# RobinWitch/SynTalker

Measured on AMD Instinct MI355X. Metric: denoising-steps/sec (128-frame clips), higher is better.
Workload: dtype bf16

## Files before the change

### include/syn_hip.h

```cpp
#ifndef SYN_HIP_H
#define SYN_HIP_H

#include <stddef.h>
#include <stdint.h>

#ifdef __cplusplus
extern "C" {
#endif

#define SYN_ABI_VERSION 9
#define SYN_D        512
#define SYN_T        32
#define SYN_C        1536
#define SYN_FF       1024
#define SYN_HEADS    4
#define SYN_LAYERS   8

int         syn_version(void);
const char* syn_last_error(void);

typedef struct syn_layer {
    const float* ln1_g;  const float* ln1_b;
    const void*  w_qkv;
    const void*  w_proj; const float* b_proj;
// ... 495 lines not shown
int syn_vq_train_wgrad(const void* dy_bf16, int32_t ldy, const void* x_bf16, int32_t ldx, float* dw, float* db, int32_t clips, int32_t t_in,
                       int32_t t_out, int32_t cout, int32_t cin, int32_t taps, int32_t stride, int32_t dil, int32_t pad, int32_t up, int32_t relu_in,
                       void* stream);
int syn_vq_train_codebook_prep(const float* codebook, float* codebook_t, float* code_sq, void* stream);
int syn_vq_train_tile(const float* x, int32_t rows, const float* noise, float* codebook, float* code_sum, float* code_count, void* stream);
int syn_vq_train_quantize(const float* x_in, const float* codebook, const float* codebook_t, const float* code_sq, const float* gumbel, float temperature,
                          float* x_out, float* q_acc, void* q_bf16, float* resid_sum, int32_t* idx, float* sqerr, int32_t layer, int32_t first, int32_t rows,
                          void* stream);
int syn_vq_train_codebook_update(const float* x_in, const int32_t* idx, int32_t layer, int32_t rows, const float* noise, float mu, float one_minus_mu,
                                 float* codebook, float* code_sum, float* code_count, float* batch_count, void* stream);
int32_t syn_vq_train_loss_parts(int64_t rows, int32_t dim_padded);
int syn_vq_train_loss(const float* rec, const float* gt, int64_t rows, int32_t dim, int32_t dim_padded, int32_t kind, void* d_rec_bf16, float* parts,
                      void* stream);
int syn_vq_train_scalars(const float* parts, int32_t n_parts, int64_t count, const float* sqerr, int32_t groups, const float* batch_count, int32_t n_active,
                         int32_t rows, float commit_weight, float* out4, void* stream);

int syn_linear(const void* x_bf16, const void* w_packed, const float* bias, int32_t m_rows, int32_t n, int32_t k, float* y,
               void* stream);
int syn_linear_and_pack(const void* x_bf16, const void* w_packed, const float* bias, int32_t m_rows, int32_t n, int32_t k, float* y,
                        void* xt_packed, void* stream);
int syn_linear_pair(const void* x1_bf16, const void* w1_packed, int32_t m1, int32_t n1, int32_t k1, float* y1,
                    const void* x2_bf16, const void* w2_packed, int32_t m2, int32_t n2, int32_t k2, float* y2,
                    const float* bias_parts, int32_t part_rows, int32_t part_n, float* bias_grad, void* stream);
int syn_linear_res(const void* x_bf16, const void* w_packed, const float* bias, const float* residual, const float* row_scale,
                   int32_t rows_per_scale, int32_t m_rows, int32_t n, int32_t k, float* y, void* xt_packed, void* stream);
int syn_linear_gelu(const void* x_bf16, const void* w_packed, const float* bias, int32_t m_rows, int32_t n, int32_t k, float* y, void* y_gelu_bf16,
                    void* xt_packed, void* stream);

int syn_test_gemm(const void* x_bf16, const void* w_packed, const float* bias, int32_t m_rows, int32_t n, int32_t k,
                  int32_t m_tile, float* y, void* stream);
int syn_test_handoff(uint32_t* sync_320_zeroed, uint32_t* buf_8x4096, const float* stream, int64_t stream_n, uint32_t* stale_9_zeroed,
                     int32_t words, int32_t rounds, int32_t mode, void* stream_h);
int syn_test_mfma_rate(int32_t iters, float* out, int64_t* flops, void* stream);
int syn_test_attention(const void* q, const void* k, const void* vt, int32_t n_seq, void* o, void* stream);

void syn_debug_timing(long long* attn_buf, long long* mlp_buf);
void syn_debug_gemm_resident(int on);
void syn_debug_linear_tile(int rows);
void syn_debug_conv_terms(int mask);
void syn_debug_seq_skew(int units_of_64_cycles);
void syn_debug_seq_step(int step);

#ifdef __cplusplus
}
#endif
#endif
```

### syntalker_amd/csrc/syn_kernels.hip

```cpp
#include <hip/hip_runtime.h>
#include <stdint.h>
#include <stdio.h>
#include <stdlib.h>
#include <string.h>

#include "syn_hip.h"

typedef __attribute__((ext_vector_type(8))) __bf16 bf16x8;
typedef __attribute__((ext_vector_type(4))) __bf16 bf16x4;
typedef __attribute__((ext_vector_type(4))) float f32x4;

#define MFMA16(a, b, c) __builtin_amdgcn_mfma_f32_16x16x32_bf16((a), (b), (c), 0, 0, 0)

namespace {

constexpr int kThreads = 512;
constexpr int kKT = 64;
constexpr int kNT = 512;

enum Epi { EPI_PLAIN = 0, EPI_IN = 1, EPI_QKV = 2, EPI_RESID = 3, EPI_GELU = 4, EPI_OUT = 5 };

struct GArgs {
    const __bf16* X; long x_chunk_stride; int ldx; int x_rows;
    const uint4* W; int K; int M;
// ... 1798 lines not shown
        hipLaunchKernelGGL((k_gemm_pair<16, 2>), grid, dim3(kThreads), lds128, (hipStream_t)stream, p);
    } else if (g_gemm_resident == 1 && fits)
        hipLaunchKernelGGL((k_gemm_pair<16, 1>), grid, dim3(kThreads), (k1 > k2 ? k1 : k2) * 32, (hipStream_t)stream, p);
    else
        hipLaunchKernelGGL((k_gemm_pair<16, 0>), grid, dim3(kThreads), 2 * 32 * 128 + 1024, (hipStream_t)stream, p);
    return launched("k_gemm_pair launch");
}

void syn_debug_gemm_resident(int on) { g_gemm_resident = on; }
void syn_debug_linear_tile(int rows) { g_linear_mt = rows; }

int syn_test_handoff(uint32_t* sync_320_zeroed, uint32_t* buf_8x4096, const float* stream, int64_t stream_n, uint32_t* stale_9_zeroed,
                     int32_t words, int32_t rounds, int32_t mode, void* stream_h) {
    if (!sync_320_zeroed || !buf_8x4096 || !stale_9_zeroed || words <= 0 || words > 4096 || rounds <= 0 || mode < 0 || mode > 4)
        return fail_msg("syn_test_handoff: bad arguments");
    if (!latency_path_ok()) return fail_msg("syn_test_handoff: needs a 256-CU (8 XCD x 32) device");
    static OncePerDevice once;
    if (once.first()) { allow_lds(lat::k_handoff_stress, 96 * 1024); }
    lat::HArgs a;
    a.sync = sync_320_zeroed; a.buf = buf_8x4096; a.stream = stream; a.stream_n = stream_n; a.stale = stale_9_zeroed;
    a.words = words; a.rounds = rounds; a.mode = mode;
    hipLaunchKernelGGL(lat::k_handoff_stress, dim3(256), dim3(512), 96 * 1024, (hipStream_t)stream_h, a);
    return launched("k_handoff_stress launch");
}

int syn_test_mfma_rate(int32_t iters, float* out, int64_t* flops, void* stream) {
    if (iters <= 0 || !out) return fail_msg("syn_test_mfma_rate: bad arguments (out: 256 floats per CU)");
    static OncePerDevice once;
    if (once.first()) { allow_lds(seq::k_mfma_rate, seq::kLds); }
    const int cus = device_cus();
    hipLaunchKernelGGL(seq::k_mfma_rate, dim3(cus), dim3(seq::kThreads), seq::kLds, (hipStream_t)stream, out, iters);
    if (flops) *flops = (int64_t)cus * 4 * (int64_t)iters * 16 * 12 * (2LL * 32 * 32 * 16);
    return launched("k_mfma_rate launch");
}

int syn_test_attention(const void* q, const void* k, const void* vt, int32_t n_seq, void* o, void* stream) {
    if (!q || !k || !vt || !o || n_seq <= 0) return fail_msg("syn_test_attention: bad arguments");
    hipLaunchKernelGGL(k_attn, dim3(n_seq), dim3(256), 0, (hipStream_t)stream, (const __bf16*)q, (const __bf16*)k,
                       (const __bf16*)vt, (__bf16*)o, n_seq);
    return launched("k_attn launch");
}

int syn_rotary(const float* x, const float* cos_t, const float* sin_t, int32_t n_seq, int32_t inverse, float* y, void* stream) {
    if (!x || !cos_t || !sin_t || !y || n_seq <= 0) return fail_msg("syn_rotary: null pointer / empty batch");
    const long n_tok = (long)n_seq * SYN_T;
    hipLaunchKernelGGL(trn::k_rotary, dim3((unsigned)((n_tok * 64 + 255) / 256)), dim3(256), 0, (hipStream_t)stream, x, cos_t, sin_t, n_tok, inverse, y);
    return launched("k_rotary launch");
}

enum { ST_IN = 0, ST_QKV = 1, ST_ATTN = 2, ST_PROJ = 3, ST_FC1 = 4, ST_FC2 = 5, ST_COMBINE = 6, ST_OUT = 7, ST_N = 8 };

struct StageTimer {
    bool on = false;
    hipStream_t s = nullptr;
    hipEvent_t ev[64];
    int cls[64];
    int n = 0;
    void begin(hipStream_t st) { on = true; s = st; hipEventCreate(&ev[0]); hipEventRecord(ev[0], s); n = 1; }
    void mark(int c) {
        if (!on || n >= 64) return;
        hipEventCreate(&ev[n]); hipEventRecord(ev[n], s); cls[n] = c; ++n;
    }
};

static int g_seq_skew = -1, g_seq_dbg_step = 0;

// ... 245 lines not shown
```

### syntalker_amd/csrc/syn_seq.inc

```
namespace {
namespace seq {

typedef __attribute__((ext_vector_type(16))) float f32x16;
#define MFMA32(a, b, c) __builtin_amdgcn_mfma_f32_32x32x16_bf16((a), (b), (c), 0, 0, 0)

#ifndef SEQ_ABL
#define SEQ_ABL 0
#endif
#ifndef SEQ_ABL2
#define SEQ_ABL2 0
#endif
constexpr int kThreads = 256;
constexpr int kFragBytes = 1024;
#ifndef SEQ_CHUNK
#define SEQ_CHUNK 16
#endif
#ifndef SEQ_WIN
#define SEQ_WIN 4
#endif
#ifndef SEQ_SPREAD
#define SEQ_SPREAD 1
#endif
#ifndef SEQ_SCHED
#define SEQ_SCHED 0
#endif
constexpr int kChunkFrags = SEQ_CHUNK, kChunkBytes = kChunkFrags * kFragBytes;
constexpr int kPerWave = kChunkFrags / 4;
constexpr int kSlots = 80 / kChunkFrags, kLook = kSlots - 1;
constexpr int kRingBytes = kSlots * kChunkBytes;
constexpr int kBiasSet = 2048;
constexpr int kRingBase = 0;
constexpr int kBiasBase = kRingBytes;
constexpr int kSlabBase = kBiasBase + 2 * kBiasSet * 4;
constexpr int kSlabBytes = 4 * 4096;
constexpr int kLds = kSlabBase + 4 * kSlabBytes;
#if SEQ_CHUNK == 16
#define SEQ_WAIT_STEADY "s_waitcnt vmcnt(8)"
#define SEQ_WAIT_FIRST "s_waitcnt vmcnt(12)"
#else
#define SEQ_WAIT_STEADY "s_waitcnt vmcnt(14)"
#define SEQ_WAIT_FIRST "s_waitcnt vmcnt(16)"
#endif

struct QArgs {
    const char* tape; unsigned tape_chunks;
    const float* bias;
    const float* te; const float* rcos; const float* rsin;
    const float* cond; const int* t_model;
    const float* xt;
    const uint4* xb;
    const float* noise;
    const unsigned long long* rng; const float* coef; const int* t_coef;
    float* xn; uint4* xnb; float* x0;
    int R;
    int V;
    const float* cfg_w;
    int cfg_stride;
    int n_steps;
    int tm_stride, tc_stride;
    int wg0, n_wg;
    int dbg_step;
    unsigned skew;
    long long* dbg;
};

__device__ __forceinline__ void dma_frag(const char* src, unsigned lds_dst, unsigned lane16) {
    unsigned keep;
    asm volatile("s_mov_b32 %0, m0\n\t"
                 "s_mov_b32 m0, %2\n\t"
                 "s_nop 0\n\t"
                 "global_load_lds_dwordx4 %1, %3\n\t"
                 "s_mov_b32 m0, %0"
                 : "=&s"(keep) : "v"(lane16), "s"(lds_dst), "s"(src) : "memory");
}

template <int OFF>
__device__ __forceinline__ void dma_frag_at(const char* src, unsigned lds_dst, unsigned lane16) {
    asm volatile("s_mov_b32 m0, %1\n\t"
                 "s_nop 0\n\t"
                 "global_load_lds_dwordx4 %0, %2 offset:%c3"
                 :: "v"(lane16), "s"(lds_dst), "s"(src), "i"(OFF) : "memory");
}

#ifndef SEQ_DMA_POL
#define SEQ_DMA_POL 0
#endif
#if SEQ_DMA_POL == 1
#define SEQ_DMA_POLICY " nt"
#elif SEQ_DMA_POL == 2
#define SEQ_DMA_POLICY " sc1"
#elif SEQ_DMA_POL == 3
#define SEQ_DMA_POLICY " sc0"
#else
#define SEQ_DMA_POLICY ""
#endif
struct Ring {
    const char* tape;
    unsigned voff;
    unsigned dst;
    unsigned wq;
    unsigned voff0;
    unsigned lane16;
    unsigned cur, nxt;
    bf16x8 win[SEQ_WIN];
};
static_assert(SEQ_CHUNK == 16 && kPerWave == 4, "the pinned ring arithmetic below is written for 16-fragment chunks");

template <int OFF>
__device__ __forceinline__ void ring_dma(const Ring& r) {
    asm volatile("s_add_u32 m0, %1, %2\n\t"
                 "s_nop 0\n\t"
                 "global_load_lds_dwordx4 %0, %3 offset:%c4" SEQ_DMA_POLICY
                 :: "v"(r.voff), "s"(r.dst), "s"(r.wq), "s"(r.tape), "i"(OFF) : "memory", "scc");
}
__device__ __forceinline__ void ring_dma_i(const Ring& r, int i) {
    switch (i) {
        case 0: ring_dma<0>(r); break;
        case 1: ring_dma<1024>(r); break;
        case 2: ring_dma<2048>(r); break;
        default: ring_dma<3072>(r); break;
    }
}
__device__ __forceinline__ void ring_advance_dma(Ring& r) {
    const unsigned d = r.dst + kChunkBytes;
    r.dst = d == (unsigned)kRingBytes ? 0u : d;
    r.voff += kChunkBytes;
}
__device__ __forceinline__ void ring_next_base(Ring& r) {
    static_assert(kSlots == 5 && kRingBase == 0, "slot arithmetic");
    unsigned t = r.dst + 2 * kChunkBytes;
    t = t >= (unsigned)kRingBytes ? t - kRingBytes : t;
    r.nxt = r.lane16 + t;
}

__device__ __forceinline__ void bias_issue(const float* bias, const Ring& r, int set) {
    const char* src = reinterpret_cast<const char*>(bias + (size_t)set * kBiasSet) + r.wq / 2;
    const unsigned dst = kBiasBase + (set & 1) * (kBiasSet * 4) + r.wq / 2;
    dma_frag(src, dst, r.lane16);
    dma_frag(src + kFragBytes, dst + kFragBytes, r.lane16);
}

__device__ __forceinline__ void ring_boundary(Ring& r) {
    if (!(SEQ_ABL & 2)) {
        if (!(SEQ_ABL & 64)) asm volatile(SEQ_WAIT_STEADY ::: "memory");
        if (!(SEQ_ABL & 128)) __builtin_amdgcn_s_barrier();
    }
    r.cur = r.nxt;
}

__device__ __forceinline__ bf16x8 take(Ring& r, const char* lds, int& f) {
    if (f == 0) {
        const bf16x8 a = r.win[0];
        if (!(SEQ_ABL & 4)) r.win[0] = *reinterpret_cast<const bf16x8*>(lds + r.nxt + SEQ_WIN * kFragBytes);
        ring_boundary(r);
        __builtin_amdgcn_sched_barrier(0);
        f = 1;
        return a;
    }
    if (!(SEQ_ABL & 1) && (f & 3) == 2) ring_dma_i(r, f >> 2);
    if (f == 6) ring_next_base(r);
    if (f == 15) ring_advance_dma(r);
    const bf16x8 a = r.win[f & (SEQ_WIN - 1)];
    const int g = f + SEQ_WIN;
    if (!(SEQ_ABL & 4))
        r.win[f & (SEQ_WIN - 1)] = *reinterpret_cast<const bf16x8*>(lds + (g < kChunkFrags ? r.cur + g * kFragBytes : r.nxt + (g - kChunkFrags) * kFragBytes));
#if SEQ_SCHED == 0
    __builtin_amdgcn_sched_barrier(0);
#else
    __builtin_amdgcn_sched_group_barrier(0x100, 1, 0);
    __builtin_amdgcn_sched_group_barrier(0x008, 1, 0);
    __builtin_amdgcn_sched_group_barrier(0x002, SEQ_SCHED, 0);
#endif
    f = (f + 1) & (kChunkFrags - 1);
    return a;
}

__device__ __forceinline__ bf16x8 pack8(const f32x16& t, int c) {
    bf16x8 o;
#pragma unroll
    for (int e = 0; e < 8; ++e) o[e] = (__bf16)t[8 * c + e];
    return o;
}

__device__ __forceinline__ f32x16 zero16() {
    f32x16 z;
#pragma unroll
    for (int v = 0; v < 16; ++v) z[v] = 0.f;
// ... 22 lines not shown
    }
    return o;
}
__device__ __forceinline__ void slab_store(char* slab, int t, const f32x16& v) {
#pragma unroll
    for (int q = 0; q < 4; ++q)
        *reinterpret_cast<f32x4*>(slab + (t * 4 + q) * 1024) = f32x4{v[4 * q], v[4 * q + 1], v[4 * q + 2], v[4 * q + 3]};
}

__device__ __forceinline__ float xor32(float v) { return __shfl_xor(v, 32); }

__device__ __forceinline__ float gelu_fast(float x) {
    if (SEQ_ABL2 & 1) return x;
    const float x2 = fminf(x * x, 64.0f);
    float t = fmaf(1.0142633e-3f, x2, -1.0677573e-1f);
    t = fmaf(t, x2, -2.3011213f);
    const float e = __builtin_amdgcn_exp2f(x * t);
    return nopk(x * __builtin_amdgcn_rcpf(1.0f + e));
}

struct NoFill { __device__ __forceinline__ void operator()(int) const {} };

__device__ __forceinline__ void slab_load_half(const char* slab, int t, int half, f32x16& o) {
#pragma unroll
    for (int q = 2 * half; q < 2 * half + 2; ++q) {
        const f32x4 v = *reinterpret_cast<const f32x4*>(slab + (t * 4 + q) * 1024);
        o[4 * q] = v[0]; o[4 * q + 1] = v[1]; o[4 * q + 2] = v[2]; o[4 * q + 3] = v[3];
    }
}
__device__ __forceinline__ void slab_store_quad(char* slab, int t, int q, const f32x16& v) {
    *reinterpret_cast<f32x4*>(slab + (t * 4 + q) * 1024) = f32x4{v[4 * q], v[4 * q + 1], v[4 * q + 2], v[4 * q + 3]};
}

template <int KC, int SPLIT = 0, typename Opnd, typename Fill = NoFill>
__device__ __forceinline__ void wide_of(Ring& r, const char* lds, f32x16 (&h)[12], char* slab, Opnd opnd, Fill fill = Fill()) {
    static_assert(SPLIT >= 0 && SPLIT < KC && (SPLIT == 0 || 12 * SPLIT >= 20), "slab loads must fit in front of their first use");
    constexpr int kLoad0 = SPLIT ? 12 * SPLIT - 12 : 0;
    constexpr int kStore0 = KC > 1 ? 16 * (KC - 1) + 4 : 16 * KC;
    f32x16 s[4];
    int f = 0, n = 0;
    auto mm = [&](f32x16& acc, int kc) {
        acc = MFMA32(take(r, lds, f), opnd(kc), acc);
        if (n >= kLoad0 && n < kLoad0 + 8) slab_load_half(slab, (n - kLoad0) >> 1, (n - kLoad0) & 1, s[(n - kLoad0) >> 1]);
        if (n >= kStore0 && n < kStore0 + 12) {
            const int j = n - kStore0, first = j < 4 ? 2 * j : 4 + j, cnt = j < 4 ? 2 : 1;
#pragma unroll
            for (int w = first; w < first + cnt; ++w) slab_store_quad(slab, w >> 2, w & 3, s[w >> 2]);
        }
        fill(n);
        ++n;
    };
    if constexpr (SPLIT > 0) {
#pragma unroll
        for (int kc = 0; kc < SPLIT; ++kc)
#pragma unroll
            for (int t = 0; t < 12; ++t) mm(h[t], kc);
#pragma unroll
        for (int kc = 0; kc < SPLIT; ++kc)
#pragma unroll
            for (int t = 0; t < 4; ++t) mm(s[t], kc);
    }
#pragma unroll
    for (int kc = SPLIT; kc < KC; ++kc) {
        if (KC > 1 && kc == KC - 1) {
#pragma unroll
            for (int t = 0; t < 4; ++t) mm(s[t], kc);
#pragma unroll
            for (int t = 0; t < 12; ++t) mm(h[t], kc);
        } else {
#pragma unroll
            for (int t = 0; t < 12; ++t) mm(h[t], kc);
#pragma unroll
            for (int t = 0; t < 4; ++t) mm(s[t], kc);
        }
    }
    if constexpr (KC == 1) {
#pragma unroll
        for (int t = 0; t < 4; ++t) slab_store(slab, t, s[t]);
    }
}

template <int KC, typename Fill = NoFill>
__device__ __forceinline__ void wide(Ring& r, const char* lds, f32x16 (&h)[12], char* slab, bf16x8 (&B)[KC], Fill fill = Fill()) {
    wide_of<KC, 0>(r, lds, h, slab, [&](int kc) { return B[kc]; }, fill);
}

template <bool SWAP, typename Fill = NoFill>
__device__ __forceinline__ void pair512(Ring& r, const char* lds, const bf16x8 (&B)[32], f32x16& a0, f32x16& a1, Fill fill = Fill()) {
    int f = 0;
#pragma unroll
    for (int kc = 0; kc < 32; ++kc) {
        const bf16x8 w0 = take(r, lds, f);
        a0 = SWAP ? MFMA32(B[kc], w0, a0) : MFMA32(w0, B[kc], a0);
        const bf16x8 w1 = take(r, lds, f);
        a1 = SWAP ? MFMA32(B[kc], w1, a1) : MFMA32(w1, B[kc], a1);
        fill(kc);
    }
}

typedef float f32x2 __attribute__((ext_vector_type(2)));
__device__ __forceinline__ f32x2 pk_add(f32x2 a, f32x2 b) { return a + b; }
__device__ __forceinline__ f32x2 pk_fma(f32x2 a, f32x2 b, f32x2 c) { return a * b + c; }

__device__ __forceinline__ void norm_to_operands(const f32x16 (&h)[12], const char* slab, bf16x8 (&xn)[32]) {
    if (SEQ_ABL2 & 16) {
#pragma unroll
        for (int i = 0; i < 32; ++i)
#pragma unroll
            for (int e = 0; e < 8; ++e) xn[i][e] = (__bf16)0.01f;
        return;
    }
    f32x2 s2 = {0.f, 0.f}, q2 = {0.f, 0.f};
#pragma unroll
    for (int t = 0; t < 16; ++t) {
        const f32x16 v = t < 12 ? h[t] : slab_load(slab, t - 12);
#pragma unroll
        for (int i = 0; i < 8; ++i) {
            const f32x2 p = {v[2 * i], v[2 * i + 1]};
            s2 = pk_add(s2, p);
            q2 = pk_fma(p, p, q2);
        }
    }
    float s = s2[0] + s2[1], q = q2[0] + q2[1];
    if (SEQ_ABL2 & 2) { s = 1.f; q = 600.f; }
    s += xor32(s); q += xor32(q);
// ... 15 lines not shown
            }
            xn[2 * t + c] = o;
        }
    }
}

using KArgs = const __attribute__((address_space(4))) QArgs;
#define KARGS(name) KArgs* name = reinterpret_cast<KArgs*>(reinterpret_cast<unsigned long long>(__builtin_amdgcn_kernarg_segment_ptr())); asm volatile("" : "+s"(name))

template <bool G, int NZ>
__global__ __launch_bounds__(kThreads) void k_seq(const QArgs) {
    extern __shared__ __attribute__((aligned(16))) char lds[];
    KARGS(a0);
    const int lane0 = threadIdx.x & 63;
    const int wave = __builtin_amdgcn_readfirstlane(threadIdx.x >> 6);
    int seq, cseq, var = 0, group0 = 0;
    bool live;
    if constexpr (!G) {
        seq = (a0->wg0 + (int)blockIdx.x) * 4 + wave;
        live = seq < a0->R;
        seq = live ? seq : a0->R - 1;
        cseq = seq;
    } else {
        const int V = a0->V, cpw = 4 / V;
        const int g = wave / V;
        seq = (a0->wg0 + (int)blockIdx.x) * cpw + g;
        live = g < cpw && seq < a0->R;
        var = live ? wave - g * V : -1;
        group0 = live ? g * V : 0;
        seq = live ? seq : a0->R - 1;
        cseq = (live ? var : 0) * a0->R + seq;
    }

    Ring r;
    r.tape = a0->tape; r.lane16 = (unsigned)lane0 * 16;
    r.wq = (unsigned)__builtin_amdgcn_readfirstlane(wave * (kPerWave * kFragBytes));
    r.voff0 = r.lane16 + r.wq;
    bias_issue(a0->bias, r, 0);
    r.voff = r.voff0; r.dst = kRingBase;
#pragma unroll 1
    for (int c = 0; c < kLook; ++c) {
#pragma unroll
        for (int i = 0; i < kPerWave; ++i) ring_dma_i(r, i);
        ring_advance_dma(r);
    }
    asm volatile(SEQ_WAIT_FIRST ::: "memory");
    __builtin_amdgcn_s_barrier();
    r.cur = r.lane16 + kRingBase;
    r.nxt = r.cur;
#pragma unroll
    for (int i = 0; i < SEQ_WIN; ++i) r.win[i] = *reinterpret_cast<const bf16x8*>(lds + kRingBase + r.lane16 + i * kFragBytes);
    if (a0->skew) {
        const unsigned n = (unsigned)(((unsigned long long)a0->skew * blockIdx.x) / gridDim.x);
        for (unsigned i = 0; i < n; ++i) __builtin_amdgcn_s_sleep(1);
        __builtin_amdgcn_s_barrier();
    }
    if (a0->dbg && wave == 0 && lane0 == 0) a0->dbg[(size_t)blockIdx.x * 32 + 0] = (long long)__builtin_readcyclecounter();

#pragma unroll 1
  for (int step = 0; step < a0->n_steps; ++step) {
    KARGS(a);
    if (step) {
        if constexpr (G) asm volatile("s_waitcnt vmcnt(0)" ::: "memory");
        __builtin_amdgcn_s_barrier();
        bias_issue(a->bias, r, 0);
        r.voff = r.voff0 + kLook * kChunkBytes;
        asm volatile("" : "+v"(r.voff));
    }
    int lane = lane0;
    asm volatile("" : "+v"(lane));
    const int hi = lane >> 5, tok = lane & 31;
    char* const slab = lds + kSlabBase + wave * kSlabBytes + lane * 16;
    const bool stamp = a->dbg && wave == 0 && lane == 0 && step == a->dbg_step;
    f32x16 h[12];
    {
        f32x16 g[16];
        const int ts = a->t_model[(size_t)step * a->tm_stride + cseq];
        const float* cp = a->cond + ((size_t)cseq * 32 + tok) * SYN_D + 4 * hi;
        const float* tp = a->te + (size_t)ts * SYN_D + 4 * hi;
#pragma unroll
        for (int t = 0; t < 16; ++t)
#pragma unroll
            for (int q = 0; q < 4; ++q) {
                const f32x4 c = *reinterpret_cast<const f32x4*>(cp + 32 * t + 8 * q);
                const f32x4 e = *reinterpret_cast<const f32x4*>(tp + 32 * t + 8 * q);
                g[t][4 * q] = c[0] + e[0]; g[t][4 * q + 1] = c[1] + e[1]; g[t][4 * q + 2] = c[2] + e[2]; g[t][4 * q + 3] = c[3] + e[3];
            }
        const uint4* xp = a->xb + (size_t)seq * (96 * 64) + lane;
        uint4 xq[8];
#pragma unroll
        for (int u = 0; u < 8; ++u) xq[u] = xp[u * 64];
#ifndef SEQ_IN_UNROLL
#define SEQ_IN_UNROLL 1
#endif
#pragma unroll SEQ_IN_UNROLL
        for (int j = 0; j < 12; ++j) {
#pragma unroll
            for (int u = 0; u < 8; ++u) {
                const bf16x8 b = __builtin_bit_cast(bf16x8, xq[u]);
                const int kn = min(j * 8 + u + 8, 95);
                if (!(SEQ_ABL & 32)) xq[u] = xp[(size_t)kn * 64];
                int f = 0;
#pragma unroll
                for (int t = 0; t < 16; ++t) g[t] = MFMA32(take(r, lds, f), b, g[t]);
            }
        }
        f32x4 cs[4], sn[4];
#pragma unroll
        for (int q = 0; q < 4; ++q) {
            cs[q] = *reinterpret_cast<const f32x4*>(a->rcos + tok * 32 + 8 * q + 4 * hi);
            sn[q] = *reinterpret_cast<const f32x4*>(a->rsin + tok * 32 + 8 * q + 4 * hi);
        }
#pragma unroll
        for (int p = 0; p < 8; ++p)
#pragma unroll
            for (int v = 0; v < 16; ++v) {
                const float u = g[2 * p][v], w = g[2 * p + 1][v], c = cs[v >> 2][v & 3], s = sn[v >> 2][v & 3];
                g[2 * p][v] = u * c - w * s;
                g[2 * p + 1][v] = w * c + u * s;
            }
#pragma unroll
        for (int t = 0; t < 12; ++t) h[t] = g[t];
#pragma unroll
        for (int t = 0; t < 4; ++t) slab_store(slab, t, g[12 + t]);
    }
    if (stamp) a->dbg[(size_t)blockIdx.x * 32 + 1] = (long long)__builtin_readcyclecounter();

    const float scale = 0.08838834764831845f * 1.4426950408889634f;
    auto make_ones = [&](bf16x8 (&o)[1]) {
        int hz = hi;
        asm volatile("" : "+v"(hz));
#pragma unroll
        for (int e = 0; e < 8; ++e) o[0][e] = (__bf16)((hz == 0 && e < 2) ? 1.0f : 0.0f);
    };
#pragma unroll 1
    for (int l = 0; l < SYN_LAYERS; ++l) {
        bf16x8 xn[32];
        norm_to_operands(h, slab, xn);
// ... 74 lines not shown
                else if (i == 32) hb[4] = pack8(b0, 0);
                else if (i == 33) hb[5] = pack8(b0, 1);
                else if (i == 34) hb[6] = pack8(b1, 0);
                else if (i == 35) hb[7] = pack8(b1, 1);
            });
        }
        if (stamp) a->dbg[(size_t)blockIdx.x * 32 + 2 + l] = (long long)__builtin_readcyclecounter();
    }

    {
        KARGS(a);
        bf16x8 hb[32];
#pragma unroll
        for (int t = 0; t < 16; ++t) {
            const f32x16 v = t < 12 ? h[t] : slab_load(slab, t - 12);
            hb[2 * t] = pack8(v, 0); hb[2 * t + 1] = pack8(v, 1);
        }
        const int tc = a->t_coef[(size_t)step * a->tc_stride + seq];
        const f32x4 cf = *reinterpret_cast<const f32x4*>(a->coef + (size_t)tc * 4);
        const size_t seq_f32 = (size_t)seq * (SYN_T * SYN_C * 4), seq_b16 = (size_t)seq * (SYN_T * SYN_C * 2);
        const char* const xt_s = reinterpret_cast<const char*>(a->xt) + seq_f32;
        char* const xn_s = reinterpret_cast<char*>(a->xn) + seq_f32;
        char* const xnb_s = reinterpret_cast<char*>(a->xnb) + seq_b16;
        char* const x0_s = a->x0 ? reinterpret_cast<char*>(a->x0) + seq_f32 : nullptr;
        [[maybe_unused]] const char* const nz_s = NZ == 1 ? reinterpret_cast<const char*>(a->noise) + seq_f32 : nullptr;
        [[maybe_unused]] unsigned long long seed = 0ull;
        [[maybe_unused]] unsigned long long idx4 = 0ull;
        if constexpr (NZ == 2) {
            seed = a->rng[0];
            idx4 = (a->rng[1] + (unsigned long long)seq) * (unsigned long long)(SYN_T * SYN_C / 4) + (unsigned long long)(tok * (SYN_C / 4) + hi);
        }
        int off_f = lane * 16, off_b = lane * 16;
        f32x16 acc_odd[2] = {zero16(), zero16()};
        f32x4 xt_odd[2][4], xo;
        [[maybe_unused]] const int nvar = G ? a->V : 1;
        [[maybe_unused]] unsigned gat = (unsigned)(kSlabBase + group0 * kSlabBytes + lane * 16);
        if constexpr (G) asm volatile("" : "+v"(gat));
        xo = f32x4{0.f, 0.f, 0.f, 0.f};
#pragma unroll
        for (int u = 0; u < 2; ++u)
#pragma unroll
            for (int q = 0; q < 4; ++q) xt_odd[u][q] = xo;
        auto fetch = [&](int off, f32x4 (&xt)[2][4]) {
#pragma unroll
            for (int u = 0; u < 2; ++u)
#pragma unroll
                for (int q = 0; q < 4; ++q)
                    xt[u][q] = (SEQ_ABL & 16) ? f32x4{1.f, 2.f, 3.f, 4.f} : *reinterpret_cast<const f32x4*>(xt_s + off + (u * 4 + q) * 1024);
        };
        auto quad = [&](int pr, int u, int q, const f32x16 (&pacc)[2], const f32x4 (&pxt)[2][4]) {
            const int at_f = off_f + (u * 4 + q) * 1024;
            f32x4 x0;
            if constexpr (!G) {
                x0 = f32x4{pacc[u][4 * q], pacc[u][4 * q + 1], pacc[u][4 * q + 2], pacc[u][4 * q + 3]};
            } else {
                const float* wc = a->cfg_w + (size_t)seq * a->cfg_stride + ((2 * pr + u) >> 4) * nvar;
                const unsigned at = gat + (unsigned)((pr & 1) * 8192 + (u * 4 + q) * 1024);
                x0 = *reinterpret_cast<const f32x4*>(lds + at) * wc[0];
#pragma unroll
                for (int v = 1; v < 4; ++v)
                    if (v < nvar) x0 = x0 + *reinterpret_cast<const f32x4*>(lds + at + v * kSlabBytes) * wc[v];
            }
            f32x4 xv;
            [[maybe_unused]] f32x4 z;
            if constexpr (NZ == 1) z = *reinterpret_cast<const f32x4*>(nz_s + at_f);
            if constexpr (NZ == 2) z = randn4<!G>(seed, (uint64_t)tc, idx4 + (unsigned long long)(8 * u + 2 * q));
#pragma unroll
            for (int e = 0; e < 4; ++e) {
                float v = fmaf(x0[e], cf[0], nopk(pxt[u][q][e] * cf[1]));
                if constexpr (NZ != 0) v = fmaf(z[e], cf[2], v);
                xv[e] = nopk(v);
            }
            if (live && (!(SEQ_ABL & 8) || a->R < 0)) {
                *reinterpret_cast<f32x4*>(xn_s + at_f) = xv;
                if (x0_s) *reinterpret_cast<f32x4*>(x0_s + at_f) = x0;
                if (q & 1) {
                    bf16x8 o;
#pragma unroll
                    for (int e = 0; e < 4; ++e) { o[e] = (__bf16)xo[e]; o[4 + e] = (__bf16)xv[e]; }
                    *reinterpret_cast<uint4*>(xnb_s + off_b + (u * 2 + (q >> 1)) * 1024) = __builtin_bit_cast(uint4, o);
                }
            }
            xo = xv;
        };
        auto advance = [&]() {
            off_f += 8192; off_b += 4096;
            if constexpr (NZ == 2) idx4 += 16;
        };
        if constexpr (!G) {
            auto pair = [&](int pr, bool first, f32x16 (&acc)[2], f32x4 (&cxt)[2][4], const f32x16 (&pacc)[2], const f32x4 (&pxt)[2][4]) {
                acc[0] = bias_tile(lds, SYN_LAYERS, 0, 2 * pr, hi); acc[1] = bias_tile(lds, SYN_LAYERS, 0, 2 * pr + 1, hi);
                fetch(first ? off_f : off_f + 8192, cxt);
                if (first) {
                    pair512<false>(r, lds, hb, acc[0], acc[1]);
                } else {
                    pair512<false>(r, lds, hb, acc[0], acc[1], [&](int kc) {
                        if ((kc & 3) == 0) quad(pr - 1, kc >> 4, (kc >> 2) & 3, pacc, pxt);
                    });
                    advance();
                }
            };
#pragma unroll 1
            for (int pp = 0; pp < 12; ++pp) {
                f32x16 acc_even[2];
                f32x4 xt_even[2][4];
                pair(2 * pp, pp == 0, acc_even, xt_even, acc_odd, xt_odd);
                pair(2 * pp + 1, false, acc_odd, xt_odd, acc_even, xt_even);
            }
        } else {
#pragma unroll 1
            for (int pr = 0; pr < 24; ++pr) {
                f32x16 acc0 = bias_tile(lds, SYN_LAYERS, 0, 2 * pr, hi), acc1 = bias_tile(lds, SYN_LAYERS, 0, 2 * pr + 1, hi);
                f32x4 cxt[2][4];
                fetch(pr == 0 ? off_f : off_f + 8192, cxt);
                if (pr == 0) {
                    pair512<false>(r, lds, hb, acc0, acc1);
                } else {
                    pair512<false>(r, lds, hb, acc0, acc1, [&](int kc) {
                        if ((kc & 3) == 0 && ((kc >> 3) % nvar) == var) quad(pr - 1, kc >> 4, (kc >> 2) & 3, acc_odd, xt_odd);
                    });
                    advance();
                }
                char* const mine = slab + (pr & 1) * 8192;
                slab_store(mine, 0, acc0);
                slab_store(mine, 1, acc1);
                asm volatile("s_waitcnt lgkmcnt(0)" ::: "memory");
#pragma unroll
                for (int u = 0; u < 2; ++u)
#pragma unroll
                    for (int q = 0; q < 4; ++q) xt_odd[u][q] = cxt[u][q];
            }
        }
        if constexpr (G) __builtin_amdgcn_s_barrier();
#pragma unroll
        for (int i = 0; i < 8; ++i)
            if (!G || ((i >> 1) % nvar) == var) quad(23, i >> 2, i & 3, acc_odd, xt_odd);
    }
    if (stamp) a->dbg[(size_t)blockIdx.x * 32 + 10] = (long long)__builtin_readcyclecounter();
  }
    if (a0->dbg && wave == 0 && lane0 == 0) a0->dbg[(size_t)blockIdx.x * 32 + 11] = (long long)__builtin_readcyclecounter();
    asm volatile("s_waitcnt vmcnt(0)" ::: "memory");
}

__global__ __launch_bounds__(256) void k_x_to_fragment(const float* __restrict__ x, float* __restrict__ of, uint4* __restrict__ ob) {
    __shared__ float tile[32][33];
    const int b = blockIdx.x, nf = blockIdx.y, tid = threadIdx.x;
#pragma unroll
    for (int i = 0; i < 4; ++i) {
        const int idx = tid + i * 256, c = idx >> 5, t = idx & 31;
        tile[c][t] = x[((size_t)b * SYN_C + 32 * nf + c) * 32 + t];
    }
    __syncthreads();
    {
        const int q = tid >> 6, lane = tid & 63, hi = lane >> 5, tk = lane & 31;
        f32x4 v;
#pragma unroll
        for (int r = 0; r < 4; ++r) v[r] = tile[8 * q + 4 * hi + r][tk];
        if (of) *reinterpret_cast<f32x4*>(of + (((size_t)b * 48 + nf) * 4 + q) * 256 + lane * 4) = v;
    }
    if (ob && tid < 128) {
        const int c = tid >> 6, lane = tid & 63, hi = lane >> 5, tk = lane & 31;
        bf16x8 o;
#pragma unroll
        for (int e = 0; e < 8; ++e) o[e] = (__bf16)tile[16 * c + 8 * (e >> 2) + 4 * hi + (e & 3)][tk];
        ob[((size_t)b * 48 + nf) * 128 + c * 64 + lane] = __builtin_bit_cast(uint4, o);
    }
}

__global__ __launch_bounds__(256) void k_x_from_fragment(const float* __restrict__ xf, float* __restrict__ out) {
// ... 50 lines not shown
```

Measured before the change: 949,400.

## Stream x_t and input fragments into LDS via async DMA interleaved with ring waits

In the non-grouped sequence kernel, x_t and the bf16 input fragments are now loaded with global_load_lds DMAs into a per-wave slab, issued in free gaps of the weight-tape ring, instead of going through per-lane global loads into registers. The ring's vmcnt waits are raised per chunk by compile-time counts of the extra DMAs outstanding, and the ring switches to a scalar source pointer. The aim is to free VGPRs and hide global load latency behind the MFMA loop. In exchange the wait-count bookkeeping is fragile and is checked only by static_asserts in a new header.

```diff
diff --git a/include/syn_hip.h b/include/syn_hip.h
--- a/include/syn_hip.h
+++ b/include/syn_hip.h
@@ -551,6 +551,7 @@
 int syn_test_handoff(uint32_t* sync_320_zeroed, uint32_t* buf_8x4096, const float* stream, int64_t stream_n, uint32_t* stale_9_zeroed,
                      int32_t words, int32_t rounds, int32_t mode, void* stream_h);
 int syn_test_mfma_rate(int32_t iters, float* out, int64_t* flops, void* stream);
+int syn_test_seq_waits(int32_t* out, int32_t n);
 int syn_test_attention(const void* q, const void* k, const void* vt, int32_t n_seq, void* o, void* stream);
 
 void syn_debug_timing(long long* attn_buf, long long* mlp_buf);
diff --git a/syntalker_amd/csrc/syn_kernels.hip b/syntalker_amd/csrc/syn_kernels.hip
--- a/syntalker_amd/csrc/syn_kernels.hip
+++ b/syntalker_amd/csrc/syn_kernels.hip
@@ -1854,6 +1854,18 @@
     hipLaunchKernelGGL(seq::k_mfma_rate, dim3(cus), dim3(seq::kThreads), seq::kLds, (hipStream_t)stream, out, iters);
     if (flops) *flops = (int64_t)cus * 4 * (int64_t)iters * 16 * 12 * (2LL * 32 * 32 * 16);
     return launched("k_mfma_rate launch");
+}
+
+int syn_test_seq_waits(int32_t* out, int32_t n) {
+    namespace w = seq::seqw;
+    if (!out || n < 32) return fail_msg("syn_test_seq_waits: out must hold 32 int32");
+    for (int i = 0; i < 32; ++i) out[i] = 0;
+    for (int i = 0; i < 4; ++i) out[i] = w::kTapeGap[i];
+    out[4] = w::kLookBack;
+    for (int i = 0; i < w::kXtFrags; ++i) out[5 + i] = w::kXtKc[i];
+    for (int c = 0; c < w::kPairChunks; ++c) { out[13 + c] = w::kOutExtra[0][c]; out[17 + c] = w::kOutExtra[1][c]; }
+    out[21] = w::kInExtra; out[22] = w::kOutTailWait;
+    return 0;
 }
 
 int syn_test_attention(const void* q, const void* k, const void* vt, int32_t n_seq, void* o, void* stream) {
diff --git a/syntalker_amd/csrc/syn_seq.inc b/syntalker_amd/csrc/syn_seq.inc
--- a/syntalker_amd/csrc/syn_seq.inc
+++ b/syntalker_amd/csrc/syn_seq.inc
@@ -41,6 +41,7 @@
 #define SEQ_WAIT_STEADY "s_waitcnt vmcnt(14)"
 #define SEQ_WAIT_FIRST "s_waitcnt vmcnt(16)"
 #endif
+#include "syn_seq_waits.inc"
 
 struct QArgs {
     const char* tape; unsigned tape_chunks;
@@ -94,8 +95,11 @@
 #else
 #define SEQ_DMA_POLICY ""
 #endif
-struct Ring {
+template <bool SP>
+struct RingT {
+    static constexpr bool kScalarPos = SP;
     const char* tape;
+    const char* src;
     unsigned voff;
     unsigned dst;
     unsigned wq;
@@ -106,13 +110,14 @@
 };
 static_assert(SEQ_CHUNK == 16 && kPerWave == 4, "the pinned ring arithmetic below is written for 16-fragment chunks");
 
-template <int OFF>
+template <int OFF, class Ring>
 __device__ __forceinline__ void ring_dma(const Ring& r) {
     asm volatile("s_add_u32 m0, %1, %2\n\t"
                  "s_nop 0\n\t"
                  "global_load_lds_dwordx4 %0, %3 offset:%c4" SEQ_DMA_POLICY
-                 :: "v"(r.voff), "s"(r.dst), "s"(r.wq), "s"(r.tape), "i"(OFF) : "memory", "scc");
-}
+                 :: "v"(Ring::kScalarPos ? r.voff0 : r.voff), "s"(r.dst), "s"(r.wq), "s"(Ring::kScalarPos ? r.src : r.tape), "i"(OFF) : "memory", "scc");
+}
+template <class Ring>
 __device__ __forceinline__ void ring_dma_i(const Ring& r, int i) {
     switch (i) {
         case 0: ring_dma<0>(r); break;
@@ -121,11 +126,13 @@
         default: ring_dma<3072>(r); break;
     }
 }
+template <class Ring>
 __device__ __forceinline__ void ring_advance_dma(Ring& r) {
     const unsigned d = r.dst + kChunkBytes;
     r.dst = d == (unsigned)kRingBytes ? 0u : d;
-    r.voff += kChunkBytes;
-}
+    if constexpr (Ring::kScalarPos) r.src += kChunkBytes; else r.voff += kChunkBytes;
+}
+template <class Ring>
 __device__ __forceinline__ void ring_next_base(Ring& r) {
     static_assert(kSlots == 5 && kRingBase == 0, "slot arithmetic");
     unsigned t = r.dst + 2 * kChunkBytes;
@@ -133,6 +140,7 @@
     r.nxt = r.lane16 + t;
 }
 
+template <class Ring>
 __device__ __forceinline__ void bias_issue(const float* bias, const Ring& r, int set) {
     const char* src = reinterpret_cast<const char*>(bias + (size_t)set * kBiasSet) + r.wq / 2;
     const unsigned dst = kBiasBase + (set & 1) * (kBiasSet * 4) + r.wq / 2;
@@ -140,19 +148,38 @@
     dma_frag(src + kFragBytes, dst + kFragBytes, r.lane16);
 }
 
-__device__ __forceinline__ void ring_boundary(Ring& r) {
+template <int N>
+__device__ __forceinline__ void wait_vm() { asm volatile("s_waitcnt vmcnt(%0)" :: "i"(N) : "memory"); }
+__device__ __forceinline__ void ring_wait(int xw) {
+    static_assert(SEQ_CHUNK == 16, "8 + xw");
+    switch (xw) {
+        case 0: asm volatile(SEQ_WAIT_STEADY ::: "memory"); break;
+        case 1: wait_vm<8 + 1>(); break;
+        case 2: wait_vm<8 + 2>(); break;
+        case 3: wait_vm<8 + 3>(); break;
+        case 4: wait_vm<8 + 4>(); break;
+        case 5: wait_vm<8 + 5>(); break;
+        case 6: wait_vm<8 + 6>(); break;
+        default: wait_vm<0>(); break;
+    }
+}
+template <class Ring>
+__device__ __forceinline__ void ring_boundary(Ring& r, int xw = 0) {
     if (!(SEQ_ABL & 2)) {
-        if (!(SEQ_ABL & 64)) asm volatile(SEQ_WAIT_STEADY ::: "memory");
+        if (!(SEQ_ABL & 64)) ring_wait(xw);
         if (!(SEQ_ABL & 128)) __builtin_amdgcn_s_barrier();
     }
     r.cur = r.nxt;
 }
 
-__device__ __forceinline__ bf16x8 take(Ring& r, const char* lds, int& f) {
+template <class Ring>
+__device__ __forceinline__ bf16x8 take(Ring& r, const char* lds, int& f, int xw = 0) {
+    static_assert(seqw::kTapeGap[0] == 2 && seqw::kTapeGap[1] == 6 && seqw::kTapeGap[2] == 10 && seqw::kTapeGap[3] == 14 && seqw::kBookGap[0] == 6 &&
+                  seqw::kBookGap[1] == 15 && seqw::kLookBack == kLook - 1, "syn_seq_waits.inc replays the gaps used below");
     if (f == 0) {
         const bf16x8 a = r.win[0];
         if (!(SEQ_ABL & 4)) r.win[0] = *reinterpret_cast<const bf16x8*>(lds + r.nxt + SEQ_WIN * kFragBytes);
-        ring_boundary(r);
+        ring_boundary(r, xw);
         __builtin_amdgcn_sched_barrier(0);
         f = 1;
         return a;
@@ -241,7 +268,7 @@
     *reinterpret_cast<f32x4*>(slab + (t * 4 + q) * 1024) = f32x4{v[4 * q], v[4 * q + 1], v[4 * q + 2], v[4 * q + 3]};
 }
 
-template <int KC, int SPLIT = 0, typename Opnd, typename Fill = NoFill>
+template <int KC, int SPLIT = 0, class Ring, typename Opnd, typename Fill = NoFill>
 __device__ __forceinline__ void wide_of(Ring& r, const char* lds, f32x16 (&h)[12], char* slab, Opnd opnd, Fill fill = Fill()) {
     static_assert(SPLIT >= 0 && SPLIT < KC && (SPLIT == 0 || 12 * SPLIT >= 20), "slab loads must fit in front of their first use");
     constexpr int kLoad0 = SPLIT ? 12 * SPLIT - 12 : 0;
@@ -289,17 +316,18 @@
     }
 }
 
-template <int KC, typename Fill = NoFill>
+template <int KC, class Ring, typename Fill = NoFill>
 __device__ __forceinline__ void wide(Ring& r, const char* lds, f32x16 (&h)[12], char* slab, bf16x8 (&B)[KC], Fill fill = Fill()) {
     wide_of<KC, 0>(r, lds, h, slab, [&](int kc) { return B[kc]; }, fill);
 }
 
-template <bool SWAP, typename Fill = NoFill>
-__device__ __forceinline__ void pair512(Ring& r, const char* lds, const bf16x8 (&B)[32], f32x16& a0, f32x16& a1, Fill fill = Fill()) {
+struct NoXw { __device__ __forceinline__ int operator()(int) const { return 0; } };
+template <bool SWAP, class Ring, typename Fill = NoFill, typename Xw = NoXw>
+__device__ __forceinline__ void pair512(Ring& r, const char* lds, const bf16x8 (&B)[32], f32x16& a0, f32x16& a1, Fill fill = Fill(), Xw xw = Xw()) {
     int f = 0;
 #pragma unroll
     for (int kc = 0; kc < 32; ++kc) {
-        const bf16x8 w0 = take(r, lds, f);
+        const bf16x8 w0 = take(r, lds, f, xw(kc >> 3));
         a0 = SWAP ? MFMA32(B[kc], w0, a0) : MFMA32(w0, B[kc], a0);
         const bf16x8 w1 = take(r, lds, f);
         a1 = SWAP ? MFMA32(B[kc], w1, a1) : MFMA32(w1, B[kc], a1);
@@ -381,12 +409,12 @@
         cseq = (live ? var : 0) * a0->R + seq;
     }
 
-    Ring r;
+    RingT<!G> r;
     r.tape = a0->tape; r.lane16 = (unsigned)lane0 * 16;
     r.wq = (unsigned)__builtin_amdgcn_readfirstlane(wave * (kPerWave * kFragBytes));
     r.voff0 = r.lane16 + r.wq;
     bias_issue(a0->bias, r, 0);
-    r.voff = r.voff0; r.dst = kRingBase;
+    r.src = r.tape; r.voff = r.voff0; r.dst = kRingBase;
 #pragma unroll 1
     for (int c = 0; c < kLook; ++c) {
 #pragma unroll
@@ -413,8 +441,12 @@
         if constexpr (G) asm volatile("s_waitcnt vmcnt(0)" ::: "memory");
         __builtin_amdgcn_s_barrier();
         bias_issue(a->bias, r, 0);
-        r.voff = r.voff0 + kLook * kChunkBytes;
-        asm volatile("" : "+v"(r.voff));
+        if constexpr (!G) {
+            r.src = a->tape + kLook * kChunkBytes;
+        } else {
+            r.voff = r.voff0 + kLook * kChunkBytes;
+            asm volatile("" : "+v"(r.voff));
+        }
     }
     int lane = lane0;
     asm volatile("" : "+v"(lane));
@@ -424,6 +456,16 @@
     f32x16 h[12];
     {
         f32x16 g[16];
+        if constexpr (!G) {
+            const char* const xb_s = reinterpret_cast<const char*>(a->xb) + (size_t)seq * (96 * kFragBytes);
+            const unsigned sdst = (unsigned)kSlabBase + 4u * r.wq;
+            if (!(SEQ_ABL & 32)) {
+                dma_frag_at<0>(xb_s, sdst, r.lane16); dma_frag_at<1024>(xb_s, sdst, r.lane16);
+                dma_frag_at<2048>(xb_s, sdst, r.lane16); dma_frag_at<3072>(xb_s, sdst, r.lane16);
+                dma_frag_at<0>(xb_s + 4096, sdst + 4096, r.lane16); dma_frag_at<1024>(xb_s + 4096, sdst + 4096, r.lane16);
+                dma_frag_at<2048>(xb_s + 4096, sdst + 4096, r.lane16); dma_frag_at<3072>(xb_s + 4096, sdst + 4096, r.lane16);
+            }
+        }
         const int ts = a->t_model[(size_t)step * a->tm_stride + cseq];
         const float* cp = a->cond + ((size_t)cseq * 32 + tok) * SYN_D + 4 * hi;
         const float* tp = a->te + (size_t)ts * SYN_D + 4 * hi;
@@ -435,6 +477,31 @@
                 const f32x4 e = *reinterpret_cast<const f32x4*>(tp + 32 * t + 8 * q);
                 g[t][4 * q] = c[0] + e[0]; g[t][4 * q + 1] = c[1] + e[1]; g[t][4 * q + 2] = c[2] + e[2]; g[t][4 * q + 3] = c[3] + e[3];
             }
+        if constexpr (!G) {
+            const char* const xb_s = reinterpret_cast<const char*>(a->xb) + (size_t)seq * (96 * kFragBytes);
+            const unsigned sdst = (unsigned)kSlabBase + 4u * r.wq;
+            asm volatile("s_waitcnt vmcnt(0)" ::: "memory");
+            auto staged = [&](int slot) {
+                return (SEQ_ABL & 256) ? r.win[slot & (SEQ_WIN - 1)] : *reinterpret_cast<const bf16x8*>(slab + slot * kFragBytes);
+            };
+            bf16x8 b = staged(0);
+            auto chunk = [&](int u, bool refill, const char* src) {
+                bf16x8 bn = b;
+                if (u < 7 || refill) bn = staged((u + 1) & 7);
+                int f = 0;
+#pragma unroll
+                for (int t = 0; t < 16; ++t) g[t] = MFMA32(take(r, lds, f, refill ? seqw::kInExtra : 0), b, g[t]);
+                if (refill && !(SEQ_ABL & 32)) dma_frag_at<0>(src + (u + seqw::kInSlots) * kFragBytes, sdst + u * kFragBytes, r.lane16);
+                b = bn;
+            };
+#pragma unroll 1
+            for (int j = 0; j < 11; ++j) {
+#pragma unroll
+                for (int u = 0; u < 8; ++u) chunk(u, true, xb_s + (size_t)j * (8 * kFragBytes));
+            }
+#pragma unroll
+            for (int u = 0; u < 8; ++u) chunk(u, false, xb_s);
+        } else {
         const uint4* xp = a->xb + (size_t)seq * (96 * 64) + lane;
         uint4 xq[8];
 #pragma unroll
@@ -453,6 +520,7 @@
 #pragma unroll
                 for (int t = 0; t < 16; ++t) g[t] = MFMA32(take(r, lds, f), b, g[t]);
             }
+        }
         }
         f32x4 cs[4], sn[4];
 #pragma unroll
@@ -593,28 +661,33 @@
         }
         int off_f = lane * 16, off_b = lane * 16;
         f32x16 acc_odd[2] = {zero16(), zero16()};
-        f32x4 xt_odd[2][4], xo;
+        [[maybe_unused]] f32x4 xt_odd[2][4];
+        f32x4 xo;
         [[maybe_unused]] const int nvar = G ? a->V : 1;
         [[maybe_unused]] unsigned gat = (unsigned)(kSlabBase + group0 * kSlabBytes + lane * 16);
         if constexpr (G) asm volatile("" : "+v"(gat));
         xo = f32x4{0.f, 0.f, 0.f, 0.f};
+        if constexpr (G) {
 #pragma unroll
         for (int u = 0; u < 2; ++u)
 #pragma unroll
             for (int q = 0; q < 4; ++q) xt_odd[u][q] = xo;
-        auto fetch = [&](int off, f32x4 (&xt)[2][4]) {
+        }
+        [[maybe_unused]] auto fetch = [&](int off, f32x4 (&xt)[2][4]) {
 #pragma unroll
             for (int u = 0; u < 2; ++u)
 #pragma unroll
                 for (int q = 0; q < 4; ++q)
                     xt[u][q] = (SEQ_ABL & 16) ? f32x4{1.f, 2.f, 3.f, 4.f} : *reinterpret_cast<const f32x4*>(xt_s + off + (u * 4 + q) * 1024);
         };
-        auto quad = [&](int pr, int u, int q, const f32x16 (&pacc)[2], const f32x4 (&pxt)[2][4]) {
+        auto quad = [&](int pr, int u, int q, const f32x16 (&pacc)[2], [[maybe_unused]] const f32x4 (*pxt)[4], [[maybe_unused]] int buf = 0) {
             const int at_f = off_f + (u * 4 + q) * 1024;
-            f32x4 x0;
+            f32x4 x0, xtv;
             if constexpr (!G) {
                 x0 = f32x4{pacc[u][4 * q], pacc[u][4 * q + 1], pacc[u][4 * q + 2], pacc[u][4 * q + 3]};
+                xtv = (SEQ_ABL & (16 | 256)) ? f32x4{1.f, 2.f, 3.f, 4.f} : *reinterpret_cast<const f32x4*>(slab + buf * 8192 + (u * 4 + q) * kFragBytes);
             } else {
+                xtv = pxt[u][q];
                 const float* wc = a->cfg_w + (size_t)seq * a->cfg_stride + ((2 * pr + u) >> 4) * nvar;
                 const unsigned at = gat + (unsigned)((pr & 1) * 8192 + (u * 4 + q) * 1024);
                 x0 = *reinterpret_cast<const f32x4*>(lds + at) * wc[0];
@@ -628,7 +701,7 @@
             if constexpr (NZ == 2) z = randn4<!G>(seed, (uint64_t)tc, idx4 + (unsigned long long)(8 * u + 2 * q));
 #pragma unroll
             for (int e = 0; e < 4; ++e) {
-                float v = fmaf(x0[e], cf[0], nopk(pxt[u][q][e] * cf[1]));
+                float v = fmaf(x0[e], cf[0], nopk(xtv[e] * cf[1]));
                 if constexpr (NZ != 0) v = fmaf(z[e], cf[2], v);
                 xv[e] = nopk(v);
             }
@@ -649,25 +722,43 @@
             if constexpr (NZ == 2) idx4 += 16;
         };
         if constexpr (!G) {
-            auto pair = [&](int pr, bool first, f32x16 (&acc)[2], f32x4 (&cxt)[2][4], const f32x16 (&pacc)[2], const f32x4 (&pxt)[2][4]) {
+            asm volatile("s_waitcnt lgkmcnt(0)" ::: "memory");
+            const unsigned sdst = (unsigned)kSlabBase + 4u * r.wq;
+            auto xt_dma = [&](int kc, int buf, bool first) {
+#pragma unroll
+                for (int i = 0; i < seqw::kXtFrags; ++i) {
+                    if (kc != seqw::kXtKc[i] || (SEQ_ABL & 16)) continue;
+                    const char* const src = xt_s + (first ? 0 : 8192) + (i & 4) * kFragBytes;
+                    const unsigned dst = sdst + buf * 8192 + (i & 4) * kFragBytes;
+                    switch (i & 3) {
+                        case 0: dma_frag_at<0>(src, dst, (unsigned)off_f); break;
+                        case 1: dma_frag_at<1024>(src, dst, (unsigned)off_f); break;
+                        case 2: dma_frag_at<2048>(src, dst, (unsigned)off_f); break;
+                        default: dma_frag_at<3072>(src, dst, (unsigned)off_f); break;
+                    }
+                }
+            };
+            constexpr bool kCount = !(SEQ_ABL & 16);
+            auto pair = [&](int pr, bool first, int buf, f32x16 (&acc)[2], const f32x16 (&pacc)[2]) {
                 acc[0] = bias_tile(lds, SYN_LAYERS, 0, 2 * pr, hi); acc[1] = bias_tile(lds, SYN_LAYERS, 0, 2 * pr + 1, hi);
-                fetch(first ? off_f : off_f + 8192, cxt);
                 if (first) {
-                    pair512<false>(r, lds, hb, acc[0], acc[1]);
+                    pair512<false>(r, lds, hb, acc[0], acc[1], [&](int kc) { xt_dma(kc, buf, true); },
+                                   [](int c) { return kCount ? seqw::kOutExtra[1][c] : 0; });
                 } else {
                     pair512<false>(r, lds, hb, acc[0], acc[1], [&](int kc) {
-                        if ((kc & 3) == 0) quad(pr - 1, kc >> 4, (kc >> 2) & 3, pacc, pxt);
-                    });
+                        if ((kc & 3) == 0) quad(pr - 1, kc >> 4, (kc >> 2) & 3, pacc, nullptr, buf ^ 1);
+                        xt_dma(kc, buf, false);
+                    }, [](int c) { return kCount ? seqw::kOutExtra[0][c] : 0; });
                     advance();
                 }
             };
 #pragma unroll 1
             for (int pp = 0; pp < 12; ++pp) {
                 f32x16 acc_even[2];
-                f32x4 xt_even[2][4];
-                pair(2 * pp, pp == 0, acc_even, xt_even, acc_odd, xt_odd);
-                pair(2 * pp + 1, false, acc_odd, xt_odd, acc_even, xt_even);
-            }
+                pair(2 * pp, pp == 0, 0, acc_even, acc_odd);
+                pair(2 * pp + 1, false, 1, acc_odd, acc_even);
+            }
+            if (kCount) wait_vm<seqw::kOutTailWait>();
         } else {
 #pragma unroll 1
             for (int pr = 0; pr < 24; ++pr) {
@@ -695,7 +786,7 @@
         if constexpr (G) __builtin_amdgcn_s_barrier();
 #pragma unroll
         for (int i = 0; i < 8; ++i)
-            if (!G || ((i >> 1) % nvar) == var) quad(23, i >> 2, i & 3, acc_odd, xt_odd);
+            if (!G || ((i >> 1) % nvar) == var) quad(23, i >> 2, i & 3, acc_odd, xt_odd, 1);
     }
     if (stamp) a->dbg[(size_t)blockIdx.x * 32 + 10] = (long long)__builtin_readcyclecounter();
   }
diff --git a/syntalker_amd/csrc/syn_seq_waits.inc b/syntalker_amd/csrc/syn_seq_waits.inc
--- /dev/null
+++ b/syntalker_amd/csrc/syn_seq_waits.inc
@@ -0,0 +1,57 @@
+namespace seqw {
+
+constexpr int kTapeGap[4] = {2, 6, 10, 14};
+constexpr int kBookGap[2] = {6, 15};
+constexpr int kLookBack = 3;
+constexpr int at(int chunk, int gap) { return 32 * chunk + 2 * gap; }
+constexpr int wait_at(int chunk) { return 32 * chunk + 1; }
+
+constexpr int kXtFrags = 8, kPairChunks = 4;
+constexpr int kXtKc[kXtFrags] = {1, 5, 9, 13, 17, 21, 25, 29};
+constexpr int xt_pos(int i) { return 2 * (2 * kXtKc[i] + 2); }
+constexpr int kInSlots = 8;
+constexpr int kInPos = at(1, 0);
+
+constexpr bool xt_schedule_ok() {
+    for (int i = 0; i < kXtFrags; ++i) {
+        const int gap = (xt_pos(i) >> 1) & 15;
+        if (gap == 0) return false;
+        for (int g : kTapeGap) if (gap == g) return false;
+        for (int g : kBookGap) if (gap == g) return false;
+        if (i && xt_pos(i) <= xt_pos(i - 1)) return false;
+        if ((xt_pos(i) >> 5) > i / 2 + kPairChunks - kLookBack) return false;
+    }
+    return true;
+}
+static_assert(xt_schedule_ok(), "x_t DMAs: free gaps only, in fragment order, each covered by a ring wait before its ds_read");
+static_assert(kTapeGap[3] == 14 && kInPos > at(0, kTapeGap[3]) && kInPos < wait_at(1), "the slot refill is younger than its period's tape DMAs and older than the next wait");
+
+constexpr int younger(const int* pos, int n, int chunks, int c, bool wrap) {
+    const int lo = at(c - kLookBack, kTapeGap[3]), hi = wait_at(c);
+    int cnt = 0;
+    for (int m = wrap ? -kLookBack : 0; m <= 0; ++m)
+        for (int i = 0; i < n; ++i) {
+            const int p = pos[i] + 32 * chunks * m;
+            if (p > lo && p < hi) ++cnt;
+        }
+    return cnt;
+}
+constexpr int kXtPos[kXtFrags] = {xt_pos(0), xt_pos(1), xt_pos(2), xt_pos(3), xt_pos(4), xt_pos(5), xt_pos(6), xt_pos(7)};
+constexpr int kInPosArr[1] = {kInPos};
+constexpr int kTapeYounger = 2 * 4;
+
+constexpr int out_extra(int c, bool first_pair) { return younger(kXtPos, kXtFrags, kPairChunks, c, !first_pair); }
+constexpr int in_extra_steady() { return younger(kInPosArr, 1, 1, 0, true); }
+constexpr int out_tail_wait() {
+    int cnt = 0;
+    for (int g : kTapeGap) if (at(kPairChunks - 1, g) > xt_pos(kXtFrags - 1)) ++cnt;
+    return cnt;
+}
+static_assert((xt_pos(kXtFrags - 1) >> 5) == kPairChunks - 1, "out_tail_wait counts the tape DMAs of the pair's last chunk");
+constexpr int kOutExtra[2][kPairChunks] = {{out_extra(0, false), out_extra(1, false), out_extra(2, false), out_extra(3, false)},
+                                           {out_extra(0, true), out_extra(1, true), out_extra(2, true), out_extra(3, true)}};
+constexpr int kInExtra = in_extra_steady();
+constexpr int kOutTailWait = out_tail_wait();
+static_assert(in_extra_steady() == 3, "one refill behind the ring's four DMAs in each of the periods k-3, k-2, k-1");
+
+}
```

Result: slower. 939,600 (-1.0%).
